# agnusmaximus/Word2Bits

Measured on AMD Instinct MI355X. Metric: training words/sec at dim=800 bitlevel=1 neg=24, higher is better.
Workload: dtype f32

## Files before the change

include/word2bits_hip.h:

```cpp
#ifndef WORD2BITS_HIP_H
#define WORD2BITS_HIP_H
#include <stdint.h>
#ifdef __cplusplus
extern "C" {
#endif

#define W2B_OK            0
#define W2B_EINVAL       -1
#define W2B_ENOGPU       -2
#define W2B_EHIP         -3
#define W2B_ENOMEM       -4
#define W2B_EUNSUPPORTED -5
#define W2B_ERCCL        -6
#define W2B_ESTATE       -7
#define W2B_EIO          -8

#define W2B_EXP_TABLE_SIZE 1000
#define W2B_MAX_EXP 6
#define W2B_MAX_SENTENCE_LENGTH 1000
#define W2B_UNIGRAM_TABLE_SIZE 100000000LL

typedef struct w2b_trainer w2b_trainer;

typedef struct w2b_config {
// ... 53 lines not shown
  int32_t exchange_tau_u;
  int32_t exchange_tau_v;
  int32_t concurrent_workers;
} w2b_tuning;
typedef struct w2b_row_plan {
  int32_t copies_u, copies_v;
  int32_t atomic_rank_u, atomic_rank_v;
  int32_t full_device;
  int32_t merge_period;
  int32_t row_group_kernel;
  int32_t refresh_rows_u;
  int32_t concurrent_workers;
} w2b_row_plan;
int w2b_plan_rows(const w2b_config *cfg, const w2b_tuning *tune, const int64_t *cn, int32_t num_cus, int32_t workers,
                  w2b_row_plan *out);
int w2b_get_tuning(w2b_trainer *t, w2b_tuning *out);
int w2b_set_tuning(w2b_trainer *t, const w2b_tuning *in);

int w2b_init_net(w2b_trainer *t);
int w2b_set_model(w2b_trainer *t, const float *u, const float *v);
int w2b_get_model(w2b_trainer *t, float *u, float *v);
int w2b_model_device_ptrs(w2b_trainer *t, void **u_dev, void **v_dev);
int w2b_export_quantized(w2b_trainer *t, float *out);
int w2b_export_packed(w2b_trainer *t, uint64_t *out);

int w2b_set_vocab_counts(w2b_trainer *t, const int64_t *cn, int64_t table_size);
int w2b_set_unigram_table(w2b_trainer *t, const int32_t *table, int64_t table_size);
int w2b_set_exp_table(w2b_trainer *t, const float *exp_table);

int w2b_set_corpus(w2b_trainer *t, const int32_t *ids, int64_t n_tokens);
// ... 47 lines not shown
```

word2bits_amd/_lib.py:

```python
import ctypes as C
import os
import sys

_HERE = os.path.dirname(os.path.abspath(__file__))
LIB_PATH = os.environ.get("W2B_LIB", os.path.join(_HERE, "libword2bits_hip.so"))

W2B_OK, W2B_EINVAL, W2B_ENOGPU, W2B_EHIP, W2B_ENOMEM = 0, -1, -2, -3, -4
W2B_EUNSUPPORTED, W2B_ERCCL, W2B_ESTATE, W2B_EIO = -5, -6, -7, -8
ERROR_NAMES = {-1: "W2B_EINVAL", -2: "W2B_ENOGPU", -3: "W2B_EHIP", -4: "W2B_ENOMEM",
               -5: "W2B_EUNSUPPORTED", -6: "W2B_ERCCL", -7: "W2B_ESTATE", -8: "W2B_EIO"}


class W2bError(RuntimeError):
    def __init__(self, code, text):
        super().__init__("%s (%d): %s" % (ERROR_NAMES.get(code, "?"), code, text))
        self.code = code


class Config(C.Structure):
    _fields_ = [
        ("vocab_size", C.c_int64), ("train_words", C.c_int64), ("iter", C.c_int64),
        ("layer1_size", C.c_int32), ("window", C.c_int32), ("negative", C.c_int32),
        ("bitlevel", C.c_int32), ("num_threads", C.c_int32),
        ("alpha", C.c_float), ("sample", C.c_float), ("reg", C.c_float),
# ... 23 lines not shown
    C.POINTER(C.c_float), C.POINTER(C.c_double)
u64p = C.POINTER(C.c_uint64)

SIGNATURES = {
    "w2b_version": (C.c_char_p, []),
    "w2b_last_error": (C.c_char_p, []),
    "w2b_device_count": (C.c_int, []),
    "w2b_device_compute_units": (C.c_int, [C.c_int32]),
    "w2b_build_exp_table": (None, [f32p]),
    "w2b_build_unigram_table": (C.c_int, [i64p, C.c_int64, i32p, C.c_int64]),
    "w2b_build_keep_prob": (None, [i64p, C.c_int64, C.c_float, C.c_int64, f32p]),
    "w2b_quantize": (C.c_float, [C.c_float, C.c_int32]),
    "w2b_trainer_create": (C.c_int, [C.POINTER(Config), C.POINTER(vp)]),
    "w2b_trainer_destroy": (None, [vp]),
    "w2b_plan_rows": (C.c_int, [C.POINTER(Config), C.POINTER(Tuning), i64p, C.c_int32, C.c_int32, C.POINTER(RowPlan)]),
    "w2b_get_tuning": (C.c_int, [vp, C.POINTER(Tuning)]),
    "w2b_set_tuning": (C.c_int, [vp, C.POINTER(Tuning)]),
    "w2b_init_net": (C.c_int, [vp]),
    "w2b_set_model": (C.c_int, [vp, f32p, f32p]),
    "w2b_get_model": (C.c_int, [vp, f32p, f32p]),
    "w2b_model_device_ptrs": (C.c_int, [vp, C.POINTER(vp), C.POINTER(vp)]),
    "w2b_export_quantized": (C.c_int, [vp, f32p]),
    "w2b_export_packed": (C.c_int, [vp, u64p]),
    "w2b_set_vocab_counts": (C.c_int, [vp, i64p, C.c_int64]),
    "w2b_set_unigram_table": (C.c_int, [vp, i32p, C.c_int64]),
    "w2b_set_exp_table": (C.c_int, [vp, f32p]),
    "w2b_set_corpus": (C.c_int, [vp, i32p, C.c_int64]),
    "w2b_set_corpus_device": (C.c_int, [vp, vp, C.c_int64]),
    "w2b_set_corpus_slice": (C.c_int, [vp, i32p, C.c_int64, C.c_int32]),
    "w2b_set_shards": (C.c_int, [vp, i64p, i32p]),
# ... 99 lines not shown
```

word2bits_amd/csrc/w2b_device.hpp:

```cpp
#pragma once
#include "w2b_internal.h"
#include <type_traits>

#ifndef W2B_T
#define W2B_T 13
#endif
#ifndef W2B_T_LOSS
#define W2B_T_LOSS W2B_T
#endif
template <bool LOSS> struct TFor { static constexpr int value = LOSS ? W2B_T_LOSS : W2B_T; };
#ifndef W2B_CA
#define W2B_CA 8
#endif
#ifndef W2B_STASH
#define W2B_STASH 8
#endif
#ifndef W2B_MINWAVES
#define W2B_MINWAVES 4
#endif

namespace {

struct QParam { int bitlevel; int steps_i; float steps_f; };

// ... 154 lines not shown
#endif

struct WordLds {
  int *ctx;
  int *umult;
  int *tgt;
  int *prev;
  int *cend;
  float *red;
  float *stash;
  float *xprod;
};

__device__ __forceinline__ int round4(int x) { return (x + 3) & ~3; }

__device__ __forceinline__ WordLds carve_word_lds(int *base, int window, int negative, int vec) {
  const int maxc = round4(2 * window + 1), maxt = round4(negative + 1);
  WordLds L;
  L.stash = reinterpret_cast<float *>(base);
  base += W2B_STASH * blockDim.x * vec;
  L.red = reinterpret_cast<float *>(base);
  int *p = base + 2 * W2B_T * W2B_MAXW;
  L.ctx = p; p += maxc;
  L.umult = p; p += maxc;
  L.tgt = p; p += maxt;
  L.prev = p; p += maxt;
  L.cend = p; p += maxt;
  L.xprod = nullptr;
  return L;
}


template <int T, typename IP>
__device__ __forceinline__ int prep_lists(IP tgt, IP prev, IP cend, int nt, IP ctx, IP umult, int cw,
                                          int lane) {
// ... 162 lines not shown
  float g;
  if (f > 6.f) g = (label - 1.f) * alpha;
  else if (f < -6.f) g = label * alpha;
  else g = (label - exp_table[(int)((f + 6.f) * 83.f)]) * alpha;
  return g;
}
__device__ __forceinline__ float log_sigmoid_term(const float f, const bool centre) {
  const float dp = centre ? f : -f;
  float sg;
  if (dp > 6.f) sg = 1.f;
  else if (dp < -6.f) sg = 1e-9f;
  else sg = 1.f / (1.f + expf(-dp));
  return logf(sg);
}

template <int QM, int VEC, bool LOSS, int MM, int ATOM = 0, int TB = -1>
__device__ __forceinline__ void process_word(const W2bParams &P, const WordLds &L, const QParam &qp,
                                             const int cw, const int nt, const float alpha,
                                             double &loss_acc, const XHot &X) {
  const int tid = threadIdx.x, lane = tid & 63, wave = tid >> 6, nwaves = blockDim.x >> 6;
  const int dim = P.dim, col0 = tid * VEC;
  const bool active = col0 < dim;
  const float ar2 = (2.f * alpha) * P.reg;
  constexpr int TC = TFor<LOSS>::value;

  Col<VEC> x[TC];
  int rows[TC];
  int start = 0, chunk = 0, end = L.cend[0];
  auto chunk_rows = [&]() {
    const int mine = L.tgt[min(start + lane, nt - 1)];
#pragma unroll
    for (int i = 0; i < TC; i++) rows[i] = __builtin_amdgcn_readlane(mine, i);
  };
  chunk_rows();
  const int nhu = (VEC == 4) ? X.nu : 0, nhv = (VEC == 4) ? X.nv : 0;
  auto ld_u = [&](int row) -> Col<VEC> {
    if constexpr (VEC == 4) { if ((unsigned)(row - 1) < (unsigned)nhu) return xhot_ld(X.cu, row - 1, nhu, dim, col0); }
    return load_col<VEC, MM, TB>(P.u, row, dim, col0, P.tab_bytes);
  };
// ... 26 lines not shown

  Col<VEC> avg;
  float regsq = 0.f;
  const bool reg_on = P.reg != 0.f;
  float *fsave = reinterpret_cast<float *>(L.prev);
#pragma unroll
  for (int e = 0; e < VEC; e++) avg.e[e] = 0.f;
  for (int j0 = 0; j0 < cw; j0 += W2B_CA) {
    Col<VEC> r[W2B_CA];
#pragma unroll
    for (int jj = 0; jj < W2B_CA; jj++)
      if (active && j0 + jj < cw) r[jj] = ld_u(__builtin_amdgcn_readfirstlane(L.ctx[j0 + jj]));
#pragma unroll
    for (int jj = 0; jj < W2B_CA; jj++)
      if (active && j0 + jj < cw) {
        if (j0 + jj < W2B_STASH) {
#pragma unroll
          for (int e = 0; e < VEC; e++) L.stash[((j0 + jj) * blockDim.x + tid) * VEC + e] = r[jj].e[e];
        }
#pragma unroll
        for (int e = 0; e < VEC; e++) {
          const float q = quant<QM>(r[jj].e[e], qp);
          avg.e[e] += q;
          if (LOSS && reg_on) regsq += q * q;
        }
      }
  }
  {
    const float cwf = (float)cw;
#pragma unroll
    for (int e = 0; e < VEC; e++) avg.e[e] = active ? avg.e[e] / cwf : 0.f;
  }

// ... 55 lines not shown
      float f = 0.f;
      for (int w = 0; w < nwaves; w++) f += red[lane * W2B_MAXW + w];
      gl = grad_scalar(f, start + lane == 0, alpha, P.exp_table);
      if (LOSS && wave == 0) fsave[start + lane] = f;
    }
#pragma unroll
    for (int i = 0; i < TC; i++) {
      if (i < n) {
        const float g = __int_as_float(__builtin_amdgcn_readlane(__float_as_int(gl), i));
        const bool by_add = (VEC == 4 && ATOM >= 2) && rows[i] <= atomic_rank && !((unsigned)(rows[i] - 1) < (unsigned)nhv);
        Col<VEC> dl;
        if constexpr (VEC == 4 && ATOM >= 2) {
#pragma unroll
          for (int e = 0; e < VEC; e++) dl.e[e] = 0.f;
        }
        if (active) {
#pragma unroll
          for (int e = 0; e < VEC; e++) {
            float xv = x[i].e[e];
            if (QM != 0) asm volatile("" : "+v"(xv));
            const float q = quant<QM>(xv, qp);
            if (LOSS && reg_on) regsq += q * q;
            err.e[e] += g * q;
            dl.e[e] = g * avg.e[e] - ar2 * xv;
            x[i].e[e] = xv + dl.e[e];
          }
          if (!by_add) up_v(rows[i], x[i], dl);
        }
        if constexpr (VEC == 4 && ATOM >= 2) {
          if (by_add) add_col_contig<TB>(P.v, rows[i], dim, dl, P.tab_bytes);
        }
      }
    }
    start = end;
    if (start >= nt) break;
    end = L.cend[++chunk];
    par ^= 1;
    chunk_rows();
    load_targets(false);
  }

  for (int j0 = 0; j0 < cw; j0 += W2B_CA) {
    Col<VEC> r[W2B_CA];
#pragma unroll
    for (int jj = 0; jj < W2B_CA; jj++)
      if (active && j0 + jj < cw && L.umult[j0 + jj] > 0) {
        const int crow = __builtin_amdgcn_readfirstlane(L.ctx[j0 + jj]);
        if (j0 + jj < W2B_STASH && crow > P.fresh_rank_u) {
#pragma unroll
          for (int e = 0; e < VEC; e++) r[jj].e[e] = L.stash[((j0 + jj) * blockDim.x + tid) * VEC + e];
        } else {
          r[jj] = ld_u(crow);
        }
      }
#pragma unroll
    for (int jj = 0; jj < W2B_CA; jj++) {
      if constexpr (VEC == 4 && ATOM >= 1) {
        if (j0 + jj < cw) {
          const int m = L.umult[j0 + jj];
          if (m > 0) {
            const int crow = __builtin_amdgcn_readfirstlane(L.ctx[j0 + jj]);
            const bool by_add = crow <= atomic_rank_u && !((unsigned)(crow - 1) < (unsigned)nhu);
            Col<VEC> dl;
#pragma unroll
            for (int e = 0; e < VEC; e++) dl.e[e] = 0.f;
            for (int k = 0; k < m; k++) {
              if (active) {
#pragma unroll
                for (int e = 0; e < VEC; e++) {
                  dl.e[e] = err.e[e] - ar2 * r[jj].e[e];
                  r[jj].e[e] = r[jj].e[e] + dl.e[e];
                }
              }
              if (by_add) add_col_contig<TB>(P.u, crow, dim, dl, P.tab_bytes);
            }
            if (!by_add && active) up_u(crow, r[jj], dl);
          }
        }
      } else {
        if (active && j0 + jj < cw) {
          const int m = L.umult[j0 + jj];
          if (m > 0) {
            const int crow = __builtin_amdgcn_readfirstlane(L.ctx[j0 + jj]);
            const bool by_add = crow <= atomic_rank_u && !(VEC == 4 && (unsigned)(crow - 1) < (unsigned)nhu);
            Col<VEC> dl;
            for (int k = 0; k < m; k++) {
#pragma unroll
              for (int e = 0; e < VEC; e++) {
                dl.e[e] = err.e[e] - ar2 * r[jj].e[e];
                r[jj].e[e] = r[jj].e[e] + dl.e[e];
              }
              if (by_add && k + 1 < m) up_u(crow, r[jj], dl);
            }
            up_u(crow, r[jj], dl);
          }
        }
      }
    }
  }
  if (LOSS) {
    if (wave == 0) {
      for (int j = lane; j < nt; j += 64) loss_acc += (double)log_sigmoid_term(fsave[j], j == 0);
    }
    if (reg_on) {
      const float s = wave_sum(active ? regsq : 0.f);
      if (lane == 0) loss_acc -= (double)(P.reg * s);
    }
  }
  __syncthreads();
// ... 232 lines not shown
    }
    const unsigned long long m = __ballot(keep);
    if (keep) tgt[1 + cnt + __popcll(m & lane_lt_mask(lane))] = t;
    cnt += __popcll(m);
  }
  if (lane == 0) tgt[0] = word;
  rng = jump_all(rng);
  return 1 + cnt;
}
template <typename JD>
__device__ __forceinline__ int table_prefetch(const W2bParams &P, const unsigned long long rng, JD jump_d, const int lane) {
  const unsigned long long xb = rng * W2B_LCG_A + W2B_LCG_C;
  return table_entry(P, jump_d(xb, lane + 1));
}

template <typename F>
hipError_t dispatch_q(int bitlevel, F &&f) {
#ifdef W2B_QUICK_BUILD
  return f(std::integral_constant<int, 1>());
#else
  switch (bitlevel) {
    case 0: return f(std::integral_constant<int, 0>());
    case 1: return f(std::integral_constant<int, 1>());
    case 2: return f(std::integral_constant<int, 2>());
    default: return f(std::integral_constant<int, 3>());
  }
#endif
}


// ... 23 lines not shown
```

word2bits_amd/csrc/w2b_internal.h:

```cpp
#pragma once
#include <hip/hip_runtime.h>
#include <stdint.h>

#define W2B_LCG_A 25214903917ULL
#define W2B_LCG_C 11ULL
#define W2B_MAX_SEN 1000
#define W2B_MAXW 16
#define W2B_NXCD 8
#define W2B_XHOT_MAX 128

struct W2bShared {
  float alpha;
  int pad0;
  unsigned long long word_count_actual;
  double loss_tuples;
  int workers_done;
  int corpus_overrun;
  unsigned long long wca_others;
  unsigned long long wca_at_sync;
  double loss_epoch;
  int launch_done, pad1;
  unsigned long long dbg[16];
};

// ... 28 lines not shown
  int mem_mode;
  float *entry;
  float *xhot;
  int xhot_u, xhot_v;
  int hot_period;
  int xhot_m;
  int uavg_rank;
  int win_refresh;
  float xhot_w;
  float *wide_scratch;
  int wide;
  int atomic_rank;
  int atomic_rank_u;
  int fresh_rank_u;
  int exact;
  int rc_rows;
  float *rc;
  int *rc_flags;
  int worker_base;
  float starting_alpha, sample, reg;
};

struct w2b_config;
struct w2b_tuning;
void w2b_shape_params(W2bParams &p, const w2b_config &cfg, const w2b_tuning &tune);

int w2b_block_threads(int dim, int *vec_out, int *wide_out = nullptr);
size_t w2b_lds_bytes(int dim, int window, int negative, bool worker_form, bool exact = false);
int w2b_tuple_max_grid(int num_cus);
hipError_t w2b_launch_tuples(const W2bParams &p, long long n, const int32_t *center,
                             const int32_t *ctx_off, const int32_t *ctx, const int32_t *neg,
                             float alpha, int grid, int num_cus, int per_cu_override, bool loss,
                             hipStream_t s);
hipError_t w2b_launch_workers(const W2bParams &p, long long max_positions, bool loss, hipStream_t s, int grid = 0);
int w2b_resident_plan(int dim, int window, int negative);
bool w2b_resident_atomic_ok(const W2bParams &p, int radius);
long long w2b_resident_scratch_rows(int radius);
hipError_t w2b_launch_resident(const W2bParams &p, long long max_positions, int radius, bool loss, hipStream_t s,
                               bool debug = false);
bool w2b_groups_ok(const W2bParams &p);
size_t w2b_groups_lds_bytes(int dim, int window, int negative);
int w2b_groups_per_cu(const W2bParams &p, bool loss);
hipError_t w2b_launch_groups(const W2bParams &p, long long max_positions, bool loss, hipStream_t s);
hipError_t w2b_launch_refresher(const W2bParams &p, hipStream_t s);
#define W2B_RC_MAX 64
#define W2B_RC_BLOCKS 16
int w2b_workers_per_cu(const W2bParams &p, bool loss);
int w2b_resident_per_cu(const W2bParams &p, int radius, bool loss);
hipError_t w2b_launch_init_net(float *u, float *v, long long n_per_table, const float *lut,
// ... 63 lines not shown
```

word2bits_amd/csrc/w2b_kernels_misc.hip:

```cpp
#include "w2b_device.hpp"

namespace {
__global__ void k_init_net(float *u, float *v, long long n, const float *__restrict__ lut) {
  const long long stride = (long long)gridDim.x * blockDim.x;
  for (long long i = (long long)blockIdx.x * blockDim.x + threadIdx.x; i < n; i += stride) {
    v[i] = lut[i & 65535];
    u[i] = lut[(n + i) & 65535];
  }
}

template <int QM>
__global__ void k_export(const float *__restrict__ u, const float *__restrict__ v, float *__restrict__ out,
                         long long n, QParam qp) {
  typedef float f4 __attribute__((ext_vector_type(4)));
  const long long stride = (long long)gridDim.x * blockDim.x;
  const bool aligned = ((((size_t)u) | ((size_t)v) | ((size_t)out)) & 15) == 0;
  const long long n4 = aligned ? (n >> 2) : 0;
  for (long long i = (long long)blockIdx.x * blockDim.x + threadIdx.x; i < n4; i += stride) {
    const f4 a = reinterpret_cast<const f4 *>(u)[i], b = reinterpret_cast<const f4 *>(v)[i];
    f4 o;
    o.x = quant<QM>(a.x + b.x, qp); o.y = quant<QM>(a.y + b.y, qp);
    o.z = quant<QM>(a.z + b.z, qp); o.w = quant<QM>(a.w + b.w, qp);
    reinterpret_cast<f4 *>(out)[i] = o;
  }
// ... 155 lines not shown
int w2b_block_threads(int dim, int *vec_out, int *wide_out) {
  int vec = (dim % 4 == 0) ? 4 : 1;
  const int cols = dim / vec;
  int threads = ((cols + 63) / 64) * 64;
  int wide = 0;
  if (threads > 1024) {
    threads = 1024;
    vec = 1;
    wide = 1;
  }
  if (vec_out) *vec_out = vec;
  if (wide_out) *wide_out = wide;
  return threads;
}

size_t w2b_lds_bytes(int dim, int window, int negative, bool worker_form, bool exact) {
  const int maxc = (2 * window + 1 + 3) & ~3, maxt = (negative + 1 + 3) & ~3;
  int vec;
  const int threads = w2b_block_threads(dim, &vec);
  size_t ints = (size_t)W2B_STASH * threads * vec + 2 * W2B_T * W2B_MAXW + 2 * maxc + 3 * maxt;
  if (worker_form) ints += ((W2B_MAX_SEN + 3) & ~3) + 4 + (sizeof(WorkerLds) + 3) / 4 + 4;
  else ints += 4;
  if (exact) ints += (size_t)W2B_T * (W2B_EXACT_COLS + 1) + 4;
  return ints * 4;
}

hipError_t w2b_launch_init_net(float *u, float *v, long long n, const float *lut, hipStream_t s) {
  hipLaunchKernelGGL(k_init_net, dim3(2048), dim3(256), 0, s, u, v, n, lut);
  return hipGetLastError();
}

hipError_t w2b_launch_export(const float *u, const float *v, float *out, long long n, int bitlevel,
                             hipStream_t s) {
  QParam qp;
  qp.bitlevel = bitlevel;
  qp.steps_i = (bitlevel >= 4) ? (1 << (bitlevel - 1)) : 1;
  qp.steps_f = (float)qp.steps_i;
  return dispatch_q(bitlevel, [&](auto qm) -> hipError_t {
    constexpr int QM = decltype(qm)::value;
// ... 56 lines not shown
```

word2bits_amd/csrc/w2b_kernels_tuples.hip:

```cpp
#include "w2b_device.hpp"

namespace {
template <int QM, int VEC, bool LOSS, int MAXTHREADS, int MM, int ATOM = 0>
__global__ void __launch_bounds__(MAXTHREADS, (MAXTHREADS <= 256 ? W2B_MINWAVES : 1)) k_train_tuples(const W2bParams P, const long long n,
                                                      const int32_t *__restrict__ center,
                                                      const int32_t *__restrict__ ctx_off,
                                                      const int32_t *__restrict__ ctx,
                                                      const int32_t *__restrict__ neg,
                                                      const float alpha) {
  extern __shared__ int smem[];
  WordLds L = carve_word_lds(smem, P.window, P.negative, VEC);
  int *s_cnt = L.cend + round4(P.negative + 1);
  if (MM == W2B_MM_EXACT) L.xprod = reinterpret_cast<float *>(s_cnt + 4);
  const int tid = threadIdx.x, lane = tid & 63;
  const bool hot = (VEC == 4 && MM == 0 && P.xhot != nullptr && P.xhot_u + P.xhot_v > 0);
  XHot XH = xhot_here(P);
  if (!hot) { XH.nu = 0; XH.nv = 0; }
  int since_merge = 0, merge_cursor = (int)(blockIdx.x >> 3) * P.xhot_m;
  const QParam qp = make_qparam(P);
  double loss_acc = 0.0;
  const int K = P.negative;
  for (long long i = blockIdx.x; i < n; i += gridDim.x) {
    if (tid < 64) {
      const int c0 = ctx_off[i], cw = ctx_off[i + 1] - c0;
      for (int j = lane; j < cw; j += 64) L.ctx[j] = ctx[c0 + j];
      const int word = center[i];
// ... 33 lines not shown
}

}

int w2b_tuple_max_grid(int num_cus) { return num_cus * 32; }
template <typename KernelT>
static int auto_grid(KernelT kernel, int threads, size_t lds, int num_cus, int per_cu_override, long long n) {
  int nb = 0;
  if (per_cu_override > 0) nb = per_cu_override;
  else if (hipOccupancyMaxActiveBlocksPerMultiprocessor(&nb, kernel, threads, lds) != hipSuccess || nb < 1) nb = 2;
  long long g = (long long)num_cus * nb;
  if (g > n) g = n;
  return (int)(g < 1 ? 1 : g);
}

hipError_t w2b_launch_tuples(const W2bParams &p, long long n, const int32_t *center, const int32_t *ctx_off,
                             const int32_t *ctx, const int32_t *neg, float alpha, int grid, int num_cus,
                             int per_cu_override, bool loss, hipStream_t s) {
  int vec;
  const int threads = w2b_block_threads(p.dim, &vec);
  const size_t lds = w2b_lds_bytes(p.dim, p.window, p.negative, false, p.exact != 0);
  return dispatch_mm_exact(p.mem_mode, p.exact, [&](auto mm) -> hipError_t {
  constexpr int MM = decltype(mm)::value;
  return dispatch_q(p.bitlevel, [&](auto qm) -> hipError_t {
    constexpr int QM = decltype(qm)::value;
#define W2B_LAUNCH_T2(VEC, LOSS, MAXT)                                                                      \
    do {                                                                                                     \
      auto kern = k_train_tuples<QM, VEC, LOSS, MAXT, MM>;                                                       \
      int g = grid > 0 ? grid : auto_grid(kern, threads, lds, num_cus, per_cu_override, n);                  \
      hipLaunchKernelGGL(kern, dim3(g), dim3(threads), lds, s, p, n, center, ctx_off, ctx, neg, alpha); \
    } while (0)
#define W2B_LAUNCH_T(VEC, LOSS) \
    do { if (threads <= 256) W2B_LAUNCH_T2(VEC, LOSS, 256); else W2B_LAUNCH_T2(VEC, LOSS, 1024); } while (0)
    if constexpr (MM == 0) {
      const int atom = p.atomic_rank > 0 ? 2 : (p.atomic_rank_u > 0 ? 1 : 0);
      if (atom && vec == 4 && threads <= 256) {
#define W2B_LAUNCH_TA(LOSS, ATOM)                                                                            \
        do {                                                                                                 \
          auto kern = k_train_tuples<QM, 4, LOSS, 256, 0, ATOM>;                                             \
          int g = grid > 0 ? grid : auto_grid(kern, threads, lds, num_cus, per_cu_override, n);              \
          hipLaunchKernelGGL(kern, dim3(g), dim3(threads), lds, s, p, n, center, ctx_off, ctx, neg, alpha);  \
        } while (0)
        if (atom == 2) { if (loss) W2B_LAUNCH_TA(true, 2); else W2B_LAUNCH_TA(false, 2); }
        else { if (loss) W2B_LAUNCH_TA(true, 1); else W2B_LAUNCH_TA(false, 1); }
#undef W2B_LAUNCH_TA
        return hipGetLastError();
      }
    }
    if (vec == 4) { if (loss) W2B_LAUNCH_T(4, true); else W2B_LAUNCH_T(4, false); }
    else { if (loss) W2B_LAUNCH_T(1, true); else W2B_LAUNCH_T(1, false); }
#undef W2B_LAUNCH_T
#undef W2B_LAUNCH_T2
    return hipGetLastError();
  });
  });
// ... 3 lines not shown
```

word2bits_amd/csrc/w2b_kernels_workers.hip:

```cpp
#include "w2b_device.hpp"

namespace {

template <int QM, int VEC, bool LOSS, int MAXTHREADS, int MM, int ATOM = 0, int TB = -1>
__global__ void __launch_bounds__(MAXTHREADS, (MAXTHREADS <= 256 ? W2B_MINWAVES : 1)) k_train_workers(const W2bParams P, const long long max_positions) {
  extern __shared__ int smem[];
  WordLds L = carve_word_lds(smem, P.window, P.negative, VEC);
  int *s_sen = L.cend + round4(P.negative + 1);
  WorkerLds *S = reinterpret_cast<WorkerLds *>(s_sen + round4(W2B_MAX_SEN) + 4);
  if (MM == W2B_MM_EXACT) L.xprod = reinterpret_cast<float *>(reinterpret_cast<int *>(S) + (sizeof(WorkerLds) + 3) / 4 + 4);
  const int tid = threadIdx.x, lane = tid & 63, wave = tid >> 6;
  const int wid = blockIdx.x + P.worker_base;
  if (wid >= P.num_threads) return;
  W2bWorker *G = P.workers + wid;
  if (G->done) return;
  const QParam qp = make_qparam(P);
  copy_sentence(s_sen, G->sen, G->sen_len, tid, blockDim.x);
  if (tid == 0) worker_restore(G, S);
  __syncthreads();
  double loss_acc = 0.0;
  const bool hot = (VEC == 4 && MM == 0 && P.xhot != nullptr && P.xhot_u + P.xhot_v > 0);
  XHot XH = xhot_here(P);
  if (!hot) { XH.nu = 0; XH.nv = 0; }
  int since_merge = 0, merge_cursor = (wid >> 3) * P.xhot_m;
// ... 36 lines not shown
      }
      if (lane == 0) {
        S->rng = rng; S->cursor = cursor; S->wc = wc; S->last_wc = last_wc;
        S->sen_len = sen_len; S->sen_pos = sen_pos; S->override_ = ovr; S->eof = eof;
        S->done = done; S->cw = cw; S->nt = nt; S->alpha = alpha;
      }
    }
    __syncthreads();
    if (S->done) break;
    const int cw = S->cw, nt = S->nt;
    const float alpha = S->alpha;
    bool wide = false;
    if constexpr (VEC == 1 && MAXTHREADS == 1024) wide = P.wide != 0;
    if (cw > 0) {
      if (wide) { if constexpr (VEC == 1 && MAXTHREADS == 1024) process_word_wide<QM, LOSS, MM>(P, L, qp, cw, nt, alpha, loss_acc); }
      else process_word<QM, VEC, LOSS, MM, ATOM, TB>(P, L, qp, cw, nt, alpha, loss_acc, XH);
    } else __syncthreads();
    if (VEC == 4 && hot && ++since_merge >= P.hot_period) {
      since_merge = 0;
      xhot_merge_event<MM, TB>(P, XH, merge_cursor, tid * VEC, tid * VEC < P.dim);
    }
  }
  __syncthreads();
  copy_sentence(G->sen, s_sen, S->sen_len, tid, blockDim.x);
  double lsum = 0.0;
  if (LOSS) {
    if (wave == 0) lsum = wave_sum_d(loss_acc);
    else if (lane == 0 && loss_acc != 0.0) { atomicAdd(&G->loss, loss_acc); atomicAdd(&P.shared->loss_epoch, loss_acc); }
  }
  if (tid == 0) {
    if (LOSS) { atomicAdd(&G->loss, lsum); atomicAdd(&P.shared->loss_epoch, lsum); }
    worker_save(P, G, S);
  }
}

}

int w2b_workers_per_cu(const W2bParams &p, bool loss) {
  int vec;
  const int threads = w2b_block_threads(p.dim, &vec);
  const size_t lds = w2b_lds_bytes(p.dim, p.window, p.negative, true, p.exact != 0);
  int nb = 0;
  (void)dispatch_mm_exact(p.mem_mode, p.exact, [&](auto mm) -> hipError_t {
    constexpr int MM = decltype(mm)::value;
    return dispatch_q(p.bitlevel, [&](auto qm) -> hipError_t {
      constexpr int QM = decltype(qm)::value;
      if (threads <= 256) return hipOccupancyMaxActiveBlocksPerMultiprocessor(&nb, k_train_workers<QM, 4, false, 256, MM>, threads, lds);
      return hipOccupancyMaxActiveBlocksPerMultiprocessor(&nb, k_train_workers<QM, 4, false, 1024, MM>, threads, lds);
    });
  });
  return nb > 0 ? nb : 1;
}

hipError_t w2b_launch_workers(const W2bParams &p, long long max_positions, bool loss, hipStream_t s, int grid) {
  if (grid <= 0) grid = p.num_threads - p.worker_base;
  int vec;
  const int threads = w2b_block_threads(p.dim, &vec);
  const size_t lds = w2b_lds_bytes(p.dim, p.window, p.negative, true, p.exact != 0);
  return dispatch_mm_exact(p.mem_mode, p.exact, [&](auto mm) -> hipError_t {
  constexpr int MM = decltype(mm)::value;
  return dispatch_q(p.bitlevel, [&](auto qm) -> hipError_t {
    constexpr int QM = decltype(qm)::value;
#define W2B_LAUNCH_W(VEC, LOSS) \
    do { if (threads <= 256) hipLaunchKernelGGL((k_train_workers<QM, VEC, LOSS, 256, MM>), dim3(grid), dim3(threads), lds, s, p, max_positions); \
         else hipLaunchKernelGGL((k_train_workers<QM, VEC, LOSS, 1024, MM>), dim3(grid), dim3(threads), lds, s, p, max_positions); } while (0)
    if constexpr (MM == 0) {
      const int atom = p.atomic_rank > 0 ? 2 : (p.atomic_rank_u > 0 ? 1 : 0);
      if (vec == 4 && threads <= 256 && (atom || p.tab_bytes != 0)) {
#define W2B_LAUNCH_A(LOSS, ATOM, TB) hipLaunchKernelGGL((k_train_workers<QM, 4, LOSS, 256, 0, ATOM, TB>), dim3(grid), dim3(threads), lds, s, p, max_positions)
#define W2B_LAUNCH_AT(LOSS, ATOM) do { if (p.tab_bytes != 0) W2B_LAUNCH_A(LOSS, ATOM, 0); else W2B_LAUNCH_A(LOSS, ATOM, -1); } while (0)
        if (atom == 2) { if (loss) W2B_LAUNCH_AT(true, 2); else W2B_LAUNCH_AT(false, 2); }
        else if (atom == 1) { if (loss) W2B_LAUNCH_AT(true, 1); else W2B_LAUNCH_AT(false, 1); }
        else { if (loss) W2B_LAUNCH_A(true, 0, 0); else W2B_LAUNCH_A(false, 0, 0); }
#undef W2B_LAUNCH_AT
#undef W2B_LAUNCH_A
        return hipGetLastError();
      }
    }
    if (vec == 4) { if (loss) W2B_LAUNCH_W(4, true); else W2B_LAUNCH_W(4, false); }
    else { if (loss) W2B_LAUNCH_W(1, true); else W2B_LAUNCH_W(1, false); }
#undef W2B_LAUNCH_W
    return hipGetLastError();
  });
  });
}
```

word2bits_amd/csrc/w2b_plan.cpp:

```cpp
#include "w2b_plan.h"

#include <cmath>

w2b_tuning w2b_default_tuning() {
  w2b_tuning tn{};
  tn.struct_size = (int32_t)sizeof(w2b_tuning);
  tn.hot_rows_v = tn.hot_rows_u = -1;
  tn.hot_period = 0;
  tn.hot_cap = 128;
  tn.force_row_desc = 0;
  tn.grid_per_cu = 0;
  tn.mem_mode = -1;
  tn.atomic_rank = -1;
  tn.atomic_cap = 0;
  tn.hot_weight_permille = 1000 / W2B_NXCD;
  tn.window_refresh = 16;
  return tn;
}

void w2b_shape_params(W2bParams &p, const w2b_config &cfg, const w2b_tuning &tune) {
  p.window_magic = cfg.window > 1 ? (unsigned long long)((((unsigned __int128)1) << 64) / (unsigned __int128)cfg.window) : 0;
  {
    const unsigned long long bytes = (unsigned long long)cfg.vocab_size * cfg.layer1_size * sizeof(float);
    p.tab_bytes = bytes < 0x7fffffffull ? (unsigned)bytes : 0u;
// ... 242 lines not shown
  in.num_cus = num_cus;
  in.tune = tune ? *tune : w2b_default_tuning();
  (void)w2b_plan_set_counts(in, cn);
  const W2bLaunchPlan lp = w2b_plan_launch(in, workers, cfg->plain_worker_kernel == 2);
  out->copies_u = lp.copies_u;
  out->copies_v = lp.copies_v;
  out->atomic_rank_v = lp.atomic_rank_v;
  out->atomic_rank_u = lp.atomic_rank_u;
  out->full_device = lp.full_device;
  out->merge_period = lp.merge_period;
  out->row_group_kernel = lp.kernel == W2B_KERNEL_GROUPS ? 1 : 0;
  out->refresh_rows_u = lp.refresh_rows_u;
  out->concurrent_workers = lp.concurrent_workers;
  return W2B_OK;
}
```

word2bits_amd/csrc/w2b_trainer.cpp:

```cpp
#include "../../include/word2bits_hip.h"
#include "../../include/word2bits_corpus.h"
#include "w2b_internal.h"
#include "w2b_plan.h"

#include <rccl/rccl.h>

#include <cmath>
#include <cstdio>
#include <cstdlib>
#include <cstring>
#include <string>
#include <vector>

static thread_local std::string g_err;
static int fail(int code, const std::string &msg) {
  g_err = msg;
  return code;
}
int w2b_internal_fail(int code, const char *msg) { return fail(code, msg ? msg : ""); }
#define HIPCHK(x)                                                                         \
  do {                                                                                    \
    hipError_t e_ = (x);                                                                  \
    if (e_ != hipSuccess)                                                                 \
      return fail(W2B_EHIP, std::string(#x) + ": " + hipGetErrorString(e_));              \
// ... 712 lines not shown
    if (int rc = rc_prepare(t, p, lp)) return rc;
    if (p.rc_rows > 0) HIPCHK(hipEventRecord(t->rc_go, t->stream));
    HIPCHK(w2b_launch_groups(p, max_positions, t->in.cfg.compute_loss != 0, t->stream));
    if (p.rc_rows > 0) {
      HIPCHK(hipStreamWaitEvent(t->rc_stream, t->rc_go, 0));
      HIPCHK(w2b_launch_refresher(p, t->rc_stream));
      HIPCHK(hipEventRecord(t->rc_end, t->rc_stream));
    }
  }
  else {
    const int conc = lp.concurrent_workers;
    W2bParams q = p;
    for (int base = 0; base < t->in.cfg.num_threads; base += conc) {
      q.worker_base = base;
      q.num_threads = t->in.cfg.num_threads;
      HIPCHK(w2b_launch_workers(q, max_positions, t->in.cfg.compute_loss != 0, t->stream, base + conc < t->in.cfg.num_threads ? conc : t->in.cfg.num_threads - base));
    }
  }
  HIPCHK(timing_end(t));
  if (p.rc_rows > 0) HIPCHK(hipStreamWaitEvent(t->stream, t->rc_end, 0));
  HIPCHK(w2b_launch_xhot_fold(p, t->stream));
  {
    if (!t->poll_host) {
      HIPCHK(hipHostMalloc((void **)&t->poll_host, sizeof(W2bShared) * w2b_trainer::kPoll, hipHostMallocDefault));
      for (int i = 0; i < w2b_trainer::kPoll; i++) HIPCHK(hipEventCreateWithFlags(&t->poll_ev[i], hipEventDisableTiming));
    }
    const int slot = (int)(t->launches % w2b_trainer::kPoll);
    HIPCHK(hipMemcpyAsync(&t->poll_host[slot], t->shared, sizeof(W2bShared), hipMemcpyDeviceToHost, t->stream));
    HIPCHK(hipEventRecord(t->poll_ev[slot], t->stream));
    t->launches++;
  }
// ... 486 lines not shown
```

Baseline: 26.19 million.

## Size LDS context stash to occupancy budget and skip unchanged row writes

```diff
diff --git a/include/word2bits_hip.h b/include/word2bits_hip.h
--- a/include/word2bits_hip.h
+++ b/include/word2bits_hip.h
@@ -91,6 +91,8 @@
 } w2b_row_plan;
 int w2b_plan_rows(const w2b_config *cfg, const w2b_tuning *tune, const int64_t *cn, int32_t num_cus, int32_t workers,
                   w2b_row_plan *out);
+int w2b_plan_stash(int32_t layer1_size, int32_t window, int32_t negative, int32_t exact_reduction, int32_t worker_form,
+                   int32_t workgroups_per_cu, int64_t lds_per_cu, int32_t *depth, int64_t *lds_bytes, int64_t *baseline_lds_bytes);
 int w2b_get_tuning(w2b_trainer *t, w2b_tuning *out);
 int w2b_set_tuning(w2b_trainer *t, const w2b_tuning *in);
 
diff --git a/word2bits_amd/_lib.py b/word2bits_amd/_lib.py
--- a/word2bits_amd/_lib.py
+++ b/word2bits_amd/_lib.py
@@ -61,6 +61,7 @@
     "w2b_trainer_create": (C.c_int, [C.POINTER(Config), C.POINTER(vp)]),
     "w2b_trainer_destroy": (None, [vp]),
     "w2b_plan_rows": (C.c_int, [C.POINTER(Config), C.POINTER(Tuning), i64p, C.c_int32, C.c_int32, C.POINTER(RowPlan)]),
+    "w2b_plan_stash": (C.c_int, [C.c_int32, C.c_int32, C.c_int32, C.c_int32, C.c_int32, C.c_int32, C.c_int64, i32p, i64p, i64p]),
     "w2b_get_tuning": (C.c_int, [vp, C.POINTER(Tuning)]),
     "w2b_set_tuning": (C.c_int, [vp, C.POINTER(Tuning)]),
     "w2b_init_net": (C.c_int, [vp]),
diff --git a/word2bits_amd/csrc/w2b_device.hpp b/word2bits_amd/csrc/w2b_device.hpp
--- a/word2bits_amd/csrc/w2b_device.hpp
+++ b/word2bits_amd/csrc/w2b_device.hpp
@@ -1,5 +1,6 @@
 #pragma once
 #include "w2b_internal.h"
+#include <string.h>
 #include <type_traits>
 
 #ifndef W2B_T
@@ -192,11 +193,12 @@
 
 __device__ __forceinline__ int round4(int x) { return (x + 3) & ~3; }
 
-__device__ __forceinline__ WordLds carve_word_lds(int *base, int window, int negative, int vec) {
+__device__ __host__ __forceinline__ int stash_cols(int dim, int vec) { return (dim + vec - 1) / vec; }
+__device__ __forceinline__ WordLds carve_word_lds(int *base, int window, int negative, int vec, int dim, int stash_depth) {
   const int maxc = round4(2 * window + 1), maxt = round4(negative + 1);
   WordLds L;
   L.stash = reinterpret_cast<float *>(base);
-  base += W2B_STASH * blockDim.x * vec;
+  base += round4(stash_depth * stash_cols(dim, vec) * vec);
   L.red = reinterpret_cast<float *>(base);
   int *p = base + 2 * W2B_T * W2B_MAXW;
   L.ctx = p; p += maxc;
@@ -389,7 +391,8 @@
   return logf(sg);
 }
 
-template <int QM, int VEC, bool LOSS, int MM, int ATOM = 0, int TB = -1>
+#define W2B_SD_FOR(MM) ((MM) == W2B_MM_EXACT ? 0 : W2B_STASH)
+template <int QM, int VEC, bool LOSS, int MM, int ATOM = 0, int TB = -1, int SD = W2B_SD_FOR(MM)>
 __device__ __forceinline__ void process_word(const W2bParams &P, const WordLds &L, const QParam &qp,
                                              const int cw, const int nt, const float alpha,
                                              double &loss_acc, const XHot &X) {
@@ -398,6 +401,10 @@
   const bool active = col0 < dim;
   const float ar2 = (2.f * alpha) * P.reg;
   constexpr int TC = TFor<LOSS>::value;
+  const int sdepth = SD > 0 ? SD : P.stash_depth, scols = stash_cols(dim, VEC);
+#ifdef W2B_PHASE_TIMERS
+  const bool timing_ = (blockIdx.x + P.worker_base == 0) && lane == 0;
+#endif
 
   Col<VEC> x[TC];
   int rows[TC];
@@ -454,9 +461,9 @@
 #pragma unroll
     for (int jj = 0; jj < W2B_CA; jj++)
       if (active && j0 + jj < cw) {
-        if (j0 + jj < W2B_STASH) {
-#pragma unroll
-          for (int e = 0; e < VEC; e++) L.stash[((j0 + jj) * blockDim.x + tid) * VEC + e] = r[jj].e[e];
+        if (j0 + jj < sdepth) {
+#pragma unroll
+          for (int e = 0; e < VEC; e++) L.stash[((j0 + jj) * scols + tid) * VEC + e] = r[jj].e[e];
         }
 #pragma unroll
         for (int e = 0; e < VEC; e++) {
@@ -542,6 +549,7 @@
 #pragma unroll
           for (int e = 0; e < VEC; e++) dl.e[e] = 0.f;
         }
+        bool changed = false;
         if (active) {
 #pragma unroll
           for (int e = 0; e < VEC; e++) {
@@ -552,11 +560,15 @@
             err.e[e] += g * q;
             dl.e[e] = g * avg.e[e] - ar2 * xv;
             x[i].e[e] = xv + dl.e[e];
+            changed = changed || __float_as_uint(x[i].e[e]) != __float_as_uint(xv);
           }
-          if (!by_add) up_v(rows[i], x[i], dl);
-        }
+        }
+        const bool any_changed = __ballot(changed) != 0ull;
+        if (wave == 0) W2B_COUNT(12);
+        if (!any_changed) W2B_COUNT(13);
+        if (active && !by_add && any_changed) up_v(rows[i], x[i], dl);
         if constexpr (VEC == 4 && ATOM >= 2) {
-          if (by_add) add_col_contig<TB>(P.v, rows[i], dim, dl, P.tab_bytes);
+          if (by_add && any_changed) add_col_contig<TB>(P.v, rows[i], dim, dl, P.tab_bytes);
         }
       }
     }
@@ -574,12 +586,14 @@
     for (int jj = 0; jj < W2B_CA; jj++)
       if (active && j0 + jj < cw && L.umult[j0 + jj] > 0) {
         const int crow = __builtin_amdgcn_readfirstlane(L.ctx[j0 + jj]);
-        if (j0 + jj < W2B_STASH && crow > P.fresh_rank_u) {
-#pragma unroll
-          for (int e = 0; e < VEC; e++) r[jj].e[e] = L.stash[((j0 + jj) * blockDim.x + tid) * VEC + e];
+        if (j0 + jj < sdepth && crow > P.fresh_rank_u) {
+#pragma unroll
+          for (int e = 0; e < VEC; e++) r[jj].e[e] = L.stash[((j0 + jj) * scols + tid) * VEC + e];
         } else {
           r[jj] = ld_u(crow);
-        }
+          if (wave == 0) W2B_COUNT(14);
+        }
+        if (wave == 0) W2B_COUNT(15);
       }
 #pragma unroll
     for (int jj = 0; jj < W2B_CA; jj++) {
@@ -590,6 +604,7 @@
             const int crow = __builtin_amdgcn_readfirstlane(L.ctx[j0 + jj]);
             const bool by_add = crow <= atomic_rank_u && !((unsigned)(crow - 1) < (unsigned)nhu);
             Col<VEC> dl;
+            bool changed = false;
 #pragma unroll
             for (int e = 0; e < VEC; e++) dl.e[e] = 0.f;
             for (int k = 0; k < m; k++) {
@@ -597,12 +612,14 @@
 #pragma unroll
                 for (int e = 0; e < VEC; e++) {
                   dl.e[e] = err.e[e] - ar2 * r[jj].e[e];
-                  r[jj].e[e] = r[jj].e[e] + dl.e[e];
+                  const float nv = r[jj].e[e] + dl.e[e];
+                  changed = changed || __float_as_uint(nv) != __float_as_uint(r[jj].e[e]);
+                  r[jj].e[e] = nv;
                 }
               }
               if (by_add) add_col_contig<TB>(P.u, crow, dim, dl, P.tab_bytes);
             }
-            if (!by_add && active) up_u(crow, r[jj], dl);
+            if (!by_add && active && __ballot(changed) != 0ull) up_u(crow, r[jj], dl);
           }
         }
       } else {
@@ -612,15 +629,18 @@
             const int crow = __builtin_amdgcn_readfirstlane(L.ctx[j0 + jj]);
             const bool by_add = crow <= atomic_rank_u && !(VEC == 4 && (unsigned)(crow - 1) < (unsigned)nhu);
             Col<VEC> dl;
+            bool changed = false;
             for (int k = 0; k < m; k++) {
 #pragma unroll
               for (int e = 0; e < VEC; e++) {
                 dl.e[e] = err.e[e] - ar2 * r[jj].e[e];
-                r[jj].e[e] = r[jj].e[e] + dl.e[e];
+                const float nv = r[jj].e[e] + dl.e[e];
+                changed = changed || __float_as_uint(nv) != __float_as_uint(r[jj].e[e]);
+                r[jj].e[e] = nv;
               }
               if (by_add && k + 1 < m) up_u(crow, r[jj], dl);
             }
-            up_u(crow, r[jj], dl);
+            if (by_add || __ballot(changed) != 0ull) up_u(crow, r[jj], dl);
           }
         }
       }
@@ -883,6 +903,41 @@
   return table_entry(P, jump_d(xb, lane + 1));
 }
 
+template <typename OCC>
+int launch_stash_depth(const W2bParams &p, bool worker_form, long long grid, int num_cus, int per_cu, OCC occ) {
+  struct Key { int dim, window, negative, exact, worker_form, mem_mode, bitlevel, num_cus, per_cu, dev; long long grid; };
+  thread_local Key have{};
+  thread_local int have_depth = -1;
+  int dev = 0;
+  (void)hipGetDevice(&dev);
+  const Key k{p.dim, p.window, p.negative, p.exact, worker_form ? 1 : 0, p.mem_mode, p.bitlevel, num_cus, per_cu, dev, grid};
+  if (have_depth >= 0 && memcmp(&k, &have, sizeof k) == 0) return have_depth;
+  int lds_cu = 0, lds_wg = 0;
+  if (hipDeviceGetAttribute(&lds_cu, hipDeviceAttributeMaxSharedMemoryPerMultiprocessor, dev) != hipSuccess || lds_cu <= 0) lds_cu = 65536;
+  if (hipDeviceGetAttribute(&lds_wg, hipDeviceAttributeMaxSharedMemoryPerBlock, dev) != hipSuccess || lds_wg <= 0) lds_wg = 65536;
+  int planned = per_cu > 0 ? per_cu : occ(w2b_lds_bytes(p.dim, p.window, p.negative, worker_form, p.exact != 0, -1));
+  if (planned < 1) planned = 1;
+  if (num_cus > 0 && grid > 0) {
+    const long long need = (grid + num_cus - 1) / num_cus > W2B_MINWAVES ? (grid + num_cus - 1) / num_cus : W2B_MINWAVES;
+    if (need < planned) planned = (int)need;
+  }
+  const long long cu = (long long)lds_wg * planned < lds_cu ? (long long)lds_wg * planned : lds_cu;
+  int depth = w2b_stash_depth(p.dim, p.window, p.negative, worker_form, p.exact != 0, planned, cu);
+  while (depth > 0 && occ(w2b_lds_bytes(p.dim, p.window, p.negative, worker_form, p.exact != 0, depth)) < planned) depth--;
+  have = k;
+  have_depth = depth;
+  return depth;
+}
+
+inline int stash_kernel_depth(int fit, int window, bool exact, bool deep, int *rows) {
+  auto need = [&](int sd) { return sd < 2 * window ? sd : 2 * window; };
+  if (exact) { *rows = fit; return 0; }
+  int sd = W2B_STASH;
+  if (deep && need(10) <= fit) sd = 10;
+  *rows = need(sd);
+  return sd;
+}
+
 template <typename F>
 hipError_t dispatch_q(int bitlevel, F &&f) {
 #ifdef W2B_QUICK_BUILD
diff --git a/word2bits_amd/csrc/w2b_internal.h b/word2bits_amd/csrc/w2b_internal.h
--- a/word2bits_amd/csrc/w2b_internal.h
+++ b/word2bits_amd/csrc/w2b_internal.h
@@ -66,6 +66,7 @@
   int atomic_rank_u;
   int fresh_rank_u;
   int exact;
+  int stash_depth;
   int rc_rows;
   float *rc;
   int *rc_flags;
@@ -78,13 +79,16 @@
 void w2b_shape_params(W2bParams &p, const w2b_config &cfg, const w2b_tuning &tune);
 
 int w2b_block_threads(int dim, int *vec_out, int *wide_out = nullptr);
-size_t w2b_lds_bytes(int dim, int window, int negative, bool worker_form, bool exact = false);
+size_t w2b_lds_bytes(int dim, int window, int negative, bool worker_form, bool exact = false, int stash_depth = -1);
+int w2b_stash_depth(int dim, int window, int negative, bool worker_form, bool exact, int wg_per_cu, long long lds_per_cu,
+                    size_t *lds_out = nullptr);
+#define W2B_LDS_GRANULE 2048
 int w2b_tuple_max_grid(int num_cus);
 hipError_t w2b_launch_tuples(const W2bParams &p, long long n, const int32_t *center,
                              const int32_t *ctx_off, const int32_t *ctx, const int32_t *neg,
                              float alpha, int grid, int num_cus, int per_cu_override, bool loss,
                              hipStream_t s);
-hipError_t w2b_launch_workers(const W2bParams &p, long long max_positions, bool loss, hipStream_t s, int grid = 0);
+hipError_t w2b_launch_workers(const W2bParams &p, long long max_positions, bool loss, hipStream_t s, int grid = 0, int num_cus = 0);
 int w2b_resident_plan(int dim, int window, int negative);
 bool w2b_resident_atomic_ok(const W2bParams &p, int radius);
 long long w2b_resident_scratch_rows(int radius);
diff --git a/word2bits_amd/csrc/w2b_kernels_misc.hip b/word2bits_amd/csrc/w2b_kernels_misc.hip
--- a/word2bits_amd/csrc/w2b_kernels_misc.hip
+++ b/word2bits_amd/csrc/w2b_kernels_misc.hip
@@ -193,15 +193,33 @@
   return threads;
 }
 
-size_t w2b_lds_bytes(int dim, int window, int negative, bool worker_form, bool exact) {
+size_t w2b_lds_bytes(int dim, int window, int negative, bool worker_form, bool exact, int stash_depth) {
   const int maxc = (2 * window + 1 + 3) & ~3, maxt = (negative + 1 + 3) & ~3;
   int vec;
   const int threads = w2b_block_threads(dim, &vec);
-  size_t ints = (size_t)W2B_STASH * threads * vec + 2 * W2B_T * W2B_MAXW + 2 * maxc + 3 * maxt;
+  const size_t stash = stash_depth < 0 ? (size_t)W2B_STASH * threads * vec
+                                       : (((size_t)stash_depth * stash_cols(dim, vec) * vec + 3) & ~(size_t)3);
+  size_t ints = stash + 2 * W2B_T * W2B_MAXW + 2 * maxc + 3 * maxt;
   if (worker_form) ints += ((W2B_MAX_SEN + 3) & ~3) + 4 + (sizeof(WorkerLds) + 3) / 4 + 4;
   else ints += 4;
   if (exact) ints += (size_t)W2B_T * (W2B_EXACT_COLS + 1) + 4;
   return ints * 4;
+}
+
+int w2b_stash_depth(int dim, int window, int negative, bool worker_form, bool exact, int wg_per_cu, long long lds_per_cu,
+                    size_t *lds_out) {
+  int vec, wide = 0;
+  (void)w2b_block_threads(dim, &vec, &wide);
+  int depth = 0;
+  if (!wide && wg_per_cu > 0) {
+    const long long budget = lds_per_cu / wg_per_cu / W2B_LDS_GRANULE * W2B_LDS_GRANULE;
+    const long long other = (long long)w2b_lds_bytes(dim, window, negative, worker_form, exact, 0);
+    const long long row = (long long)stash_cols(dim, vec) * vec * 4;
+    const long long fit = budget - other - 12 > 0 ? (budget - other - 12) / row : 0;
+    depth = (int)(fit < 2ll * window ? fit : 2ll * window);
+  }
+  if (lds_out) *lds_out = w2b_lds_bytes(dim, window, negative, worker_form, exact, depth);
+  return depth;
 }
 
 hipError_t w2b_launch_init_net(float *u, float *v, long long n, const float *lut, hipStream_t s) {
diff --git a/word2bits_amd/csrc/w2b_kernels_tuples.hip b/word2bits_amd/csrc/w2b_kernels_tuples.hip
--- a/word2bits_amd/csrc/w2b_kernels_tuples.hip
+++ b/word2bits_amd/csrc/w2b_kernels_tuples.hip
@@ -9,7 +9,7 @@
                                                       const int32_t *__restrict__ neg,
                                                       const float alpha) {
   extern __shared__ int smem[];
-  WordLds L = carve_word_lds(smem, P.window, P.negative, VEC);
+  WordLds L = carve_word_lds(smem, P.window, P.negative, VEC, P.dim, P.stash_depth);
   int *s_cnt = L.cend + round4(P.negative + 1);
   if (MM == W2B_MM_EXACT) L.xprod = reinterpret_cast<float *>(s_cnt + 4);
   const int tid = threadIdx.x, lane = tid & 63;
@@ -73,12 +73,27 @@
   return (int)(g < 1 ? 1 : g);
 }
 
-hipError_t w2b_launch_tuples(const W2bParams &p, long long n, const int32_t *center, const int32_t *ctx_off,
+hipError_t w2b_launch_tuples(const W2bParams &p_in, long long n, const int32_t *center, const int32_t *ctx_off,
                              const int32_t *ctx, const int32_t *neg, float alpha, int grid, int num_cus,
                              int per_cu_override, bool loss, hipStream_t s) {
   int vec;
-  const int threads = w2b_block_threads(p.dim, &vec);
-  const size_t lds = w2b_lds_bytes(p.dim, p.window, p.negative, false, p.exact != 0);
+  const int threads = w2b_block_threads(p_in.dim, &vec);
+  W2bParams p = p_in;
+  p.stash_depth = launch_stash_depth(p, false, grid > 0 ? (long long)grid : 0, num_cus, grid > 0 ? 0 : per_cu_override, [&](size_t lds) {
+    int nb = 0;
+    (void)dispatch_mm_exact(p.mem_mode, p.exact, [&](auto mm) -> hipError_t {
+      constexpr int MM = decltype(mm)::value;
+      return dispatch_q(p.bitlevel, [&](auto qm) -> hipError_t {
+        constexpr int QM = decltype(qm)::value;
+        if (threads <= 256) return hipOccupancyMaxActiveBlocksPerMultiprocessor(&nb, k_train_tuples<QM, 4, false, 256, MM>, threads, lds);
+        return hipOccupancyMaxActiveBlocksPerMultiprocessor(&nb, k_train_tuples<QM, 4, false, 1024, MM>, threads, lds);
+      });
+    });
+    return nb > 0 ? nb : 0;
+  });
+  (void)stash_kernel_depth(p.stash_depth, p.window, p.exact != 0, false, &p.stash_depth);
+  const size_t lds_base = w2b_lds_bytes(p.dim, p.window, p.negative, false, p.exact != 0);
+  const size_t lds = w2b_lds_bytes(p.dim, p.window, p.negative, false, p.exact != 0, p.stash_depth);
   return dispatch_mm_exact(p.mem_mode, p.exact, [&](auto mm) -> hipError_t {
   constexpr int MM = decltype(mm)::value;
   return dispatch_q(p.bitlevel, [&](auto qm) -> hipError_t {
@@ -86,7 +101,7 @@
 #define W2B_LAUNCH_T2(VEC, LOSS, MAXT)                                                                      \
     do {                                                                                                     \
       auto kern = k_train_tuples<QM, VEC, LOSS, MAXT, MM>;                                                       \
-      int g = grid > 0 ? grid : auto_grid(kern, threads, lds, num_cus, per_cu_override, n);                  \
+      int g = grid > 0 ? grid : auto_grid(kern, threads, lds_base, num_cus, per_cu_override, n);                  \
       hipLaunchKernelGGL(kern, dim3(g), dim3(threads), lds, s, p, n, center, ctx_off, ctx, neg, alpha); \
     } while (0)
 #define W2B_LAUNCH_T(VEC, LOSS) \
@@ -97,7 +112,7 @@
 #define W2B_LAUNCH_TA(LOSS, ATOM)                                                                            \
         do {                                                                                                 \
           auto kern = k_train_tuples<QM, 4, LOSS, 256, 0, ATOM>;                                             \
-          int g = grid > 0 ? grid : auto_grid(kern, threads, lds, num_cus, per_cu_override, n);              \
+          int g = grid > 0 ? grid : auto_grid(kern, threads, lds_base, num_cus, per_cu_override, n);              \
           hipLaunchKernelGGL(kern, dim3(g), dim3(threads), lds, s, p, n, center, ctx_off, ctx, neg, alpha);  \
         } while (0)
         if (atom == 2) { if (loss) W2B_LAUNCH_TA(true, 2); else W2B_LAUNCH_TA(false, 2); }
diff --git a/word2bits_amd/csrc/w2b_kernels_workers.hip b/word2bits_amd/csrc/w2b_kernels_workers.hip
--- a/word2bits_amd/csrc/w2b_kernels_workers.hip
+++ b/word2bits_amd/csrc/w2b_kernels_workers.hip
@@ -2,10 +2,10 @@
 
 namespace {
 
-template <int QM, int VEC, bool LOSS, int MAXTHREADS, int MM, int ATOM = 0, int TB = -1>
+template <int QM, int VEC, bool LOSS, int MAXTHREADS, int MM, int ATOM = 0, int TB = -1, int SD = W2B_SD_FOR(MM)>
 __global__ void __launch_bounds__(MAXTHREADS, (MAXTHREADS <= 256 ? W2B_MINWAVES : 1)) k_train_workers(const W2bParams P, const long long max_positions) {
   extern __shared__ int smem[];
-  WordLds L = carve_word_lds(smem, P.window, P.negative, VEC);
+  WordLds L = carve_word_lds(smem, P.window, P.negative, VEC, P.dim, P.stash_depth);
   int *s_sen = L.cend + round4(P.negative + 1);
   WorkerLds *S = reinterpret_cast<WorkerLds *>(s_sen + round4(W2B_MAX_SEN) + 4);
   if (MM == W2B_MM_EXACT) L.xprod = reinterpret_cast<float *>(reinterpret_cast<int *>(S) + (sizeof(WorkerLds) + 3) / 4 + 4);
@@ -74,7 +74,7 @@
     if constexpr (VEC == 1 && MAXTHREADS == 1024) wide = P.wide != 0;
     if (cw > 0) {
       if (wide) { if constexpr (VEC == 1 && MAXTHREADS == 1024) process_word_wide<QM, LOSS, MM>(P, L, qp, cw, nt, alpha, loss_acc); }
-      else process_word<QM, VEC, LOSS, MM, ATOM, TB>(P, L, qp, cw, nt, alpha, loss_acc, XH);
+      else process_word<QM, VEC, LOSS, MM, ATOM, TB, SD>(P, L, qp, cw, nt, alpha, loss_acc, XH);
     } else __syncthreads();
     if (VEC == 4 && hot && ++since_merge >= P.hot_period) {
       since_merge = 0;
@@ -96,10 +96,9 @@
 
 }
 
-int w2b_workers_per_cu(const W2bParams &p, bool loss) {
+static int workers_occupancy(const W2bParams &p, size_t lds) {
   int vec;
   const int threads = w2b_block_threads(p.dim, &vec);
-  const size_t lds = w2b_lds_bytes(p.dim, p.window, p.negative, true, p.exact != 0);
   int nb = 0;
   (void)dispatch_mm_exact(p.mem_mode, p.exact, [&](auto mm) -> hipError_t {
     constexpr int MM = decltype(mm)::value;
@@ -109,14 +108,23 @@
       return hipOccupancyMaxActiveBlocksPerMultiprocessor(&nb, k_train_workers<QM, 4, false, 1024, MM>, threads, lds);
     });
   });
+  return nb > 0 ? nb : 0;
+}
+
+int w2b_workers_per_cu(const W2bParams &p, bool loss) {
+  const int nb = workers_occupancy(p, w2b_lds_bytes(p.dim, p.window, p.negative, true, p.exact != 0));
   return nb > 0 ? nb : 1;
 }
 
-hipError_t w2b_launch_workers(const W2bParams &p, long long max_positions, bool loss, hipStream_t s, int grid) {
-  if (grid <= 0) grid = p.num_threads - p.worker_base;
+hipError_t w2b_launch_workers(const W2bParams &p_in, long long max_positions, bool loss, hipStream_t s, int grid, int num_cus) {
+  if (grid <= 0) grid = p_in.num_threads - p_in.worker_base;
   int vec;
-  const int threads = w2b_block_threads(p.dim, &vec);
-  const size_t lds = w2b_lds_bytes(p.dim, p.window, p.negative, true, p.exact != 0);
+  const int threads = w2b_block_threads(p_in.dim, &vec);
+  W2bParams p = p_in;
+  const bool deep = !p.exact && p.mem_mode == 0 && vec == 4 && threads <= 256 && p.atomic_rank <= 0 && p.atomic_rank_u <= 0 && p.tab_bytes != 0;
+  const int sd = stash_kernel_depth(launch_stash_depth(p, true, grid, num_cus, 0, [&](size_t lds) { return workers_occupancy(p, lds); }),
+                                    p.window, p.exact != 0, deep, &p.stash_depth);
+  const size_t lds = w2b_lds_bytes(p.dim, p.window, p.negative, true, p.exact != 0, p.stash_depth);
   return dispatch_mm_exact(p.mem_mode, p.exact, [&](auto mm) -> hipError_t {
   constexpr int MM = decltype(mm)::value;
   return dispatch_q(p.bitlevel, [&](auto qm) -> hipError_t {
@@ -128,11 +136,14 @@
       const int atom = p.atomic_rank > 0 ? 2 : (p.atomic_rank_u > 0 ? 1 : 0);
       if (vec == 4 && threads <= 256 && (atom || p.tab_bytes != 0)) {
 #define W2B_LAUNCH_A(LOSS, ATOM, TB) hipLaunchKernelGGL((k_train_workers<QM, 4, LOSS, 256, 0, ATOM, TB>), dim3(grid), dim3(threads), lds, s, p, max_positions)
+#define W2B_LAUNCH_D(LOSS, SD) hipLaunchKernelGGL((k_train_workers<QM, 4, LOSS, 256, 0, 0, 0, SD>), dim3(grid), dim3(threads), lds, s, p, max_positions)
 #define W2B_LAUNCH_AT(LOSS, ATOM) do { if (p.tab_bytes != 0) W2B_LAUNCH_A(LOSS, ATOM, 0); else W2B_LAUNCH_A(LOSS, ATOM, -1); } while (0)
         if (atom == 2) { if (loss) W2B_LAUNCH_AT(true, 2); else W2B_LAUNCH_AT(false, 2); }
         else if (atom == 1) { if (loss) W2B_LAUNCH_AT(true, 1); else W2B_LAUNCH_AT(false, 1); }
+        else if (sd == 10) { if (loss) W2B_LAUNCH_D(true, 10); else W2B_LAUNCH_D(false, 10); }
         else { if (loss) W2B_LAUNCH_A(true, 0, 0); else W2B_LAUNCH_A(false, 0, 0); }
 #undef W2B_LAUNCH_AT
+#undef W2B_LAUNCH_D
 #undef W2B_LAUNCH_A
         return hipGetLastError();
       }
diff --git a/word2bits_amd/csrc/w2b_plan.cpp b/word2bits_amd/csrc/w2b_plan.cpp
--- a/word2bits_amd/csrc/w2b_plan.cpp
+++ b/word2bits_amd/csrc/w2b_plan.cpp
@@ -280,3 +280,15 @@
   out->concurrent_workers = lp.concurrent_workers;
   return W2B_OK;
 }
+
+extern "C" int w2b_plan_stash(int32_t layer1_size, int32_t window, int32_t negative, int32_t exact_reduction, int32_t worker_form,
+                              int32_t workgroups_per_cu, int64_t lds_per_cu, int32_t *depth, int64_t *lds_bytes, int64_t *baseline_lds_bytes) {
+  if (layer1_size < 1 || window < 1 || negative < 0 || workgroups_per_cu < 1 || lds_per_cu < 1)
+    return w2b_internal_fail(W2B_EINVAL, "w2b_plan_stash: bad argument");
+  size_t lds = 0;
+  const int d = w2b_stash_depth(layer1_size, window, negative, worker_form != 0, exact_reduction != 0, workgroups_per_cu, lds_per_cu, &lds);
+  if (depth) *depth = d;
+  if (lds_bytes) *lds_bytes = (int64_t)lds;
+  if (baseline_lds_bytes) *baseline_lds_bytes = (int64_t)w2b_lds_bytes(layer1_size, window, negative, worker_form != 0, exact_reduction != 0, -1);
+  return W2B_OK;
+}
diff --git a/word2bits_amd/csrc/w2b_trainer.cpp b/word2bits_amd/csrc/w2b_trainer.cpp
--- a/word2bits_amd/csrc/w2b_trainer.cpp
+++ b/word2bits_amd/csrc/w2b_trainer.cpp
@@ -750,7 +750,7 @@
     for (int base = 0; base < t->in.cfg.num_threads; base += conc) {
       q.worker_base = base;
       q.num_threads = t->in.cfg.num_threads;
-      HIPCHK(w2b_launch_workers(q, max_positions, t->in.cfg.compute_loss != 0, t->stream, base + conc < t->in.cfg.num_threads ? conc : t->in.cfg.num_threads - base));
+      HIPCHK(w2b_launch_workers(q, max_positions, t->in.cfg.compute_loss != 0, t->stream, base + conc < t->in.cfg.num_threads ? conc : t->in.cfg.num_threads - base, t->in.num_cus));
     }
   }
   HIPCHK(timing_end(t));
```

After: 24.46 million. 0.934x the previous value.
